# justinkay/coda

Hardware: NVIDIA H100
Metric: acquisition steps/sec (M=256,N=5e5,C=100) (higher is better)
Workload: dtype f32

## Files before the change

coda_b200/_native.py:

```python
from __future__ import annotations

import ctypes as C
import os
import sys

from . import build as _build

_LIB = None

OK = 0
VERSION = 202
MAX_WORLD = 16
REC_WORDS = 8
FLAG_NONFINITE_INPUT = 0x01
FLAG_RANGE_INPUT = 0x02
FLAG_NONFINITE_TABLE = 0x04
FLAG_NONFINITE_PI = 0x08
FLAG_NONFINITE_PBEST = 0x10
FLAG_NONFINITE_EIG = 0x20
FLAG_NO_CANDIDATE = 0x40
FLAG_XCHG_TIMEOUT = 0x80
FLAG_NEGATIVE_PROB = 0x100
FLAG_ROWSUM_WARN = 0x200
FLAG_PIPELINE_TIMEOUT = 0x400
FLAG_NAMES = {
    FLAG_NONFINITE_INPUT: "preds", FLAG_RANGE_INPUT: "preds range", FLAG_NONFINITE_TABLE: "pdf/cdf/integrand",
    FLAG_NONFINITE_PI: "pi_hat_xi", FLAG_NONFINITE_PBEST: "Pbest", FLAG_NONFINITE_EIG: "Pbest(beta) normalized",
}

p, i32, i64, f64, f32, sz = C.c_void_p, C.c_int, C.c_int64, C.c_double, C.c_float, C.c_size_t


class XchgStruct(C.Structure):
    _fields_ = [("world", i32), ("rank", i32), ("box", p * MAX_WORLD), ("epoch", p), ("H", i32), ("C", i32),
                ("rep_words", i32)]


class StepStruct(C.Structure):
    _fields_ = [
        ("H", i32), ("C", i32), ("N", i64), ("n_offset", i64), ("fx_shift", i32), ("lr", f32),
        ("hard", p), ("labeled", p), ("D", p), ("jvec", p), ("sel", p),
        ("terms", p), ("slot_of_model", p), ("shadow_off", i64), ("shadow_col_stride", i64), ("model_stride", i64),
        ("have_ens", i32), ("compact_k", i32),
        ("pisum_fx", p), ("PB", p), ("pi_hat", p), ("m0", p), ("h_before", p), ("best_model", p),
        ("partials", p), ("nblocks", i32), ("eig", p), ("bestrec", p),
        ("labels_global", p), ("hist_idx", p), ("hist_q", p), ("hist_tie", p), ("hist_cap", i64), ("step_ctr", p),
        ("flags", p),
    ]


PX, PS = C.POINTER(XchgStruct), C.POINTER(StepStruct)

SIGNATURES = {
    "coda_b200_last_error": (C.c_char_p, []),
    "coda_b200_version": (i32, []),
    "coda_b200_sm_count": (i32, []),
    "coda_b200_device_check": (i32, []),
    "coda_b200_set_l2_fetch_granularity": (i32, [i32]),
    "coda_b200_xchg_box_bytes": (sz, [i32, i32, i32, i32]),
    "coda_b200_xchg_alloc": (i32, [sz, C.POINTER(p)]),
    "coda_b200_xchg_free": (i32, [p]),
    "coda_b200_ipc_export": (i32, [p, p]),
    "coda_b200_ipc_open": (i32, [p, C.POINTER(p)]),
    "coda_b200_ipc_close": (i32, [p]),
    "coda_b200_peer_enable": (i32, [i32]),
    "coda_b200_scan_slab": (i32, [p, i64, i32, i64, i32, p, p, p, p, p, p]),
    "coda_b200_confusion_accum": (i32, [p, i64, p, i32, i64, i32, i32, p, p]),
    "coda_b200_confusion_sorted": (i32, [p, i64, p, p, i32, i64, i32, i32, p, p]),
    "coda_b200_init_dirichlets": (i32, [p, p, i32, i32, i32, f64, f64, i32, p, p]),
    "coda_b200_scan_compact": (i32, [p, p, i64, i32, i64, i32, i32, p, p, p, p, p, p]),
    "coda_b200_confusion_compact": (i32, [p, p, i64, p, i32, i64, i32, i32, i32, p, p, p]),
    "coda_b200_pi_full_compact": (i32, [p, p, i64, p, i32, i64, i32, i32, p, p, p, p]),
    "coda_b200_pi_rank1_compact": (i32, [p, p, i64, p, i32, i64, i32, i32, p, f64, i32, p, p, p, p, p]),
    "coda_b200_compact_index_count": (i32, [p, i64, i32, i64, i32, i32, p, p]),
    "coda_b200_compact_index_fill": (i32, [p, p, i64, i32, i64, i32, i32, p, p, p, p]),
    "coda_b200_pi_rank1_index": (i32, [p, p, p, p, i32, i64, i32, p, f64, i32, p, p, p, p, p, p]),
# ... 87 lines not shown
```

coda_b200/csrc/slab.cu:

```cuda
#include "common.cuh"
#include "terms.cuh"

#include <stdlib.h>

__global__ void __launch_bounds__(256) k_scan_slab(const float* __restrict__ preds, long long ldh, int H, long long N, int C,
                                                   int TN, uint16_t* __restrict__ hard,
                                                   int32_t* __restrict__ pseudo, uint8_t* __restrict__ disagree,
                                                   float* __restrict__ ens_out, uint32_t* __restrict__ flags) {
  extern __shared__ __align__(16) unsigned char smem_raw[];
  float* ens = reinterpret_cast<float*>(smem_raw);
  uint16_t* hard_t = reinterpret_cast<uint16_t*>(ens + (size_t)TN * C);
  const int warp = threadIdx.x >> 5, lane = threadIdx.x & 31, nwarp = blockDim.x >> 5;
  const long long n0 = (long long)blockIdx.x * TN;
  const int tn = (int)min((long long)TN, N - n0);
  for (int i = threadIdx.x; i < TN * C; i += blockDim.x) ens[i] = 0.f;
  __syncthreads();
  uint32_t bad = 0;
  for (int h = 0; h < H; ++h) {
    const float* base = preds + (size_t)h * ldh + (size_t)n0 * C;
    for (int p = warp; p < tn; p += nwarp) {
      const float* row = base + (size_t)p * C;
      float* erow = ens + (size_t)p * C;
      float bv = -INFINITY;
      int bi = 0x7fffffff;
// ... 542 lines not shown
    for (int k = 0; k < KC; ++k) {
      const int c = lane + 32 * k;
      u[r][k] = (ok && c < C) ? urow[c] : 0.f;
    }
  }
#pragma unroll
  for (int r = 0; r < NR; ++r) {
    if (r * rstride >= nrows) break;
    float* urow = U + (size_t)(row0 + r * rstride) * C;
    float s = 0.f;
#pragma unroll
    for (int k = 0; k < KC; ++k) {
      const int c = lane + 32 * k;
      if (c == t) {
        u[r][k] += dv[r];
        urow[c] = u[r][k];
      }
      s += u[r][k];
    }
    s = warp_sum(s);
    if (!isfinite(s)) bad |= CODA_B200_FLAG_NONFINITE_PI;
    const float den = fmaxf(s, 1e-12f);
    const float rden = 1.0f / den;
#pragma unroll
    for (int k = 0; k < KC; ++k) racc[k] += to_fx(row_quot(u[r][k], den, rden), fxs);
  }
}

#define R1_CONST_TERMS 3584
__constant__ R1Term c_terms_bank[R1_CONST_TERMS];

#define R1_TN 256
template <int KC, int GU = 16, int NR = 4, bool CONST_TERMS = false>
__global__ void __launch_bounds__(256, (GU > 16 ? 3 : 4)) k_pi_rank1(const float* __restrict__ preds, const float* __restrict__ E,
                                                  long long N, int C, const long long* __restrict__ sel,
                                                  const int32_t* __restrict__ hdr, const R1Term* __restrict__ gterms,
                                                  int const_base, float lr, float fxs,
                                                  float* __restrict__ U, unsigned long long* __restrict__ pisum_fx,
                                                  uint32_t* __restrict__ flags) {
  extern __shared__ __align__(16) unsigned char smem_raw[];
  long long* wacc_all = reinterpret_cast<long long*>(smem_raw);
  R1Term* s_terms = reinterpret_cast<R1Term*>(wacc_all + (size_t)8 * C);
  const int warp = threadIdx.x >> 5, lane = threadIdx.x & 31;
  const int t = (int)sel[1];
  const int nt = hdr[0], tp = hdr[1];
  if (!CONST_TERMS)
    for (int k = threadIdx.x; k < nt; k += blockDim.x) s_terms[k] = gterms[k];
  const R1Term* c_terms = CONST_TERMS ? (c_terms_bank + const_base) : s_terms;
  long long* wacc = wacc_all + (size_t)warp * C;
  for (int c = lane; c < C; c += 32) wacc[c] = 0;
  long long racc[KC > 0 ? KC : 1];
#pragma unroll
  for (int k = 0; k < (KC > 0 ? KC : 1); ++k) racc[k] = 0;
  __syncthreads();
  uint32_t bad = 0;
  const long long wstride = (long long)gridDim.x * R1_TN;
  for (long long n0 = (long long)blockIdx.x * R1_TN + warp * 32; n0 < N; n0 += wstride) {
    const long long n = n0 + lane;
    float d = 0.f;
    if (n < N) {
      if (tp >= 0) d = __ldg(E + (size_t)n * C + tp);
      int k = 0;
      for (; k + GU <= nt; k += GU) {
        float v[GU];
#pragma unroll
        for (int q = 0; q < GU; ++q) v[q] = __ldg(preds + c_terms[k + q].off + n * c_terms[k + q].str);
#pragma unroll
        for (int q = 0; q < GU; ++q) d = fmaf(c_terms[k + q].sg, v[q], d);
      }
      for (; k < nt; ++k) d = fmaf(c_terms[k].sg, __ldg(preds + c_terms[k].off + n * c_terms[k].str), d);
    }
    const float dl = lr * d;
    const int rows = (int)min(32LL, N - n0);
    if (KC > 0) {
      for (int r = 0; r < rows; r += NR) {
        float dv[NR];
#pragma unroll
        for (int i = 0; i < NR; ++i) dv[i] = __shfl_sync(CODA_FULL, dl, (r + i) & 31);
        rows_accumulate_reg<(KC > 0 ? KC : 1), NR>(U, n0 + r, rows - r, 1, C, lane, fxs, t, dv, racc, bad);
      }
    } else {
      for (int r = 0; r < rows; ++r) {
        const float dr = __shfl_sync(CODA_FULL, dl, r);
        row_accumulate(U + (size_t)(n0 + r) * C, C, lane, fxs, t, dr, nullptr, wacc, bad);
      }
    }
  }
  if (KC > 0) {
#pragma unroll
    for (int k = 0; k < (KC > 0 ? KC : 1); ++k) {
      const int c = lane + 32 * k;
      if (c < C) wacc[c] = racc[k];
    }
  }
  __syncthreads();
  for (int c = threadIdx.x; c < C; c += blockDim.x) {
    long long s2 = 0;
    for (int w = 0; w < 8; ++w) s2 += wacc_all[(size_t)w * C + c];
    if (s2) atomicAdd(pisum_fx + c, (unsigned long long)s2);
  }
  if (bad) atomicOr(flags, bad);
}

#define R1V_WI 128
template <int KC>
__global__ void __launch_bounds__(256, 3) k_pi_rank1_v4(const float* __restrict__ preds, const float* __restrict__ E,
                                                     long long N, int C, const long long* __restrict__ sel,
                                                     const int32_t* __restrict__ hdr, const R1Term* __restrict__ gterms,
                                                     float lr, float fxs, float* __restrict__ U,
                                                     unsigned long long* __restrict__ pisum_fx,
                                                     uint32_t* __restrict__ flags) {
  extern __shared__ __align__(16) unsigned char smem_raw[];
  long long* wacc_all = reinterpret_cast<long long*>(smem_raw);
  R1Term* c_terms = reinterpret_cast<R1Term*>(wacc_all + (size_t)8 * C);
  const int warp = threadIdx.x >> 5, lane = threadIdx.x & 31;
  const int t = (int)sel[1];
  const int nt = hdr[0], tp = hdr[1];
  for (int k = threadIdx.x; k < nt; k += blockDim.x) c_terms[k] = gterms[k];
  long long racc[KC];
#pragma unroll
  for (int k = 0; k < KC; ++k) racc[k] = 0;
  __syncthreads();
  uint32_t bad = 0;
  const long long cta_items = (long long)8 * R1V_WI;
  for (long long n0 = (long long)blockIdx.x * cta_items + (long long)warp * R1V_WI; n0 < N; n0 += (long long)gridDim.x * cta_items) {
    const long long nl = n0 + 4 * lane;
    const bool full4 = nl + 3 < N;
    float d[4] = {0.f, 0.f, 0.f, 0.f};
    if (tp >= 0) {
#pragma unroll
      for (int i = 0; i < 4; ++i)
        if (nl + i < N) d[i] = __ldg(E + (size_t)(nl + i) * C + tp);
    }
    int k = 0;
    for (; k + 8 <= nt; k += 8) {
      float v[8][4];
#pragma unroll
      for (int q = 0; q < 8; ++q) {
        const R1Term tm = c_terms[k + q];
        if (tm.str == 1 && full4) {
          const float4 x = __ldg(reinterpret_cast<const float4*>(preds + tm.off + nl));
          v[q][0] = x.x; v[q][1] = x.y; v[q][2] = x.z; v[q][3] = x.w;
        } else {
#pragma unroll
          for (int i = 0; i < 4; ++i) v[q][i] = (nl + i < N) ? __ldg(preds + tm.off + (nl + i) * tm.str) : 0.f;
        }
      }
#pragma unroll
      for (int q = 0; q < 8; ++q) {
        const float sg = c_terms[k + q].sg;
#pragma unroll
        for (int i = 0; i < 4; ++i) d[i] = fmaf(sg, v[q][i], d[i]);
      }
    }
    for (; k < nt; ++k) {
      const R1Term tm = c_terms[k];
#pragma unroll
      for (int i = 0; i < 4; ++i) {
        const float x = (nl + i < N) ? __ldg(preds + tm.off + (nl + i) * tm.str) : 0.f;
        d[i] = fmaf(tm.sg, x, d[i]);
      }
    }
    float dl[4];
#pragma unroll
    for (int i = 0; i < 4; ++i) dl[i] = lr * d[i];
    const int rows = (int)min((long long)R1V_WI, N - n0);
    for (int r = 0; r < rows; r += 4) {
      float dv[4];
#pragma unroll
      for (int i = 0; i < 4; ++i) dv[i] = __shfl_sync(CODA_FULL, dl[i], r >> 2);
      rows_accumulate_reg<KC, 4>(U, n0 + r, rows - r, 1, C, lane, fxs, t, dv, racc, bad);
    }
  }
  long long* wacc = wacc_all + (size_t)warp * C;
#pragma unroll
  for (int k = 0; k < KC; ++k) {
    const int c = lane + 32 * k;
    if (c < C) wacc[c] = racc[k];
  }
  __syncthreads();
  for (int c = threadIdx.x; c < C; c += blockDim.x) {
    long long s2 = 0;
    for (int w = 0; w < 8; ++w) s2 += wacc_all[(size_t)w * C + c];
    if (s2) atomicAdd(pisum_fx + c, (unsigned long long)s2);
  }
  if (bad) atomicOr(flags, bad);
}

#define R1X_THREADS 320
#define R1X_ST 4
#define R1X_TB 16

template <int KC>
__global__ void __launch_bounds__(R1X_THREADS, 1) k_pi_rank1_tma(const float* __restrict__ preds,
                                                                 const float* __restrict__ E, long long N, int C, int TR,
                                                                 const long long* __restrict__ sel,
                                                                 const int32_t* __restrict__ hdr,
                                                                 const R1Term* __restrict__ gterms, float lr, float fxs,
                                                                 float* __restrict__ U,
                                                                 unsigned long long* __restrict__ pisum_fx,
                                                                 uint32_t* __restrict__ flags) {
  extern __shared__ __align__(128) unsigned char smem_r1x[];
  unsigned char* smem_raw = smem_r1x;
  const int nt = hdr[0], tp = hdr[1];
  const int t = (int)sel[1];
  const size_t u_bytes = ((size_t)TR * C * 4 + 127) & ~(size_t)127;
  float* Ut = reinterpret_cast<float*>(smem_raw);
  float* ring = reinterpret_cast<float*>(smem_raw + u_bytes);
  R1Term* terms = reinterpret_cast<R1Term*>(ring + (size_t)R1X_ST * R1X_TB * TR);
  long long* wacc_all = reinterpret_cast<long long*>(terms + nt);
  int* shl = reinterpret_cast<int*>(wacc_all + (size_t)8 * C);
  uint64_t* bars = reinterpret_cast<uint64_t*>((reinterpret_cast<uintptr_t>(shl + nt) + 7) & ~(uintptr_t)7);
  uint64_t* fullU = bars, *emptyU = bars + 1, *full = bars + 2, *empty = bars + 2 + R1X_ST;
  __shared__ int s_nsh;
  const int tid = threadIdx.x, warp = tid >> 5, lane = tid & 31;
  const int nwarp_act = TR >> 5;
  for (int k = tid; k < nt; k += R1X_THREADS) terms[k] = gterms[k];
  for (int c = tid; c < 8 * C; c += R1X_THREADS) wacc_all[c] = 0;
  if (tid == 0) {
    mbar_init(fullU, 1);
    mbar_init(emptyU, nwarp_act);
    for (int s = 0; s < R1X_ST; ++s) { mbar_init(&full[s], 1); mbar_init(&empty[s], nwarp_act); }
    mbar_fence_init();
  }
  __syncthreads();
  if (tid == 0) {
    int n = 0;
    for (int k = 0; k < nt; ++k)
      if (terms[k].str == 1) shl[n++] = k;
    s_nsh = n;
  }
  __syncthreads();
  const int nsh = s_nsh;
  const int nch = (nsh + R1X_TB - 1) / R1X_TB;
  const long long ntiles = (N + TR - 1) / TR;

  if (warp == 8) {
// ... 12 lines not shown
            tma_load_1d(ring + ((size_t)s * R1X_TB + j) * TR, preds + terms[shl[c * R1X_TB + j]].off + n0, rb, &full[s]);
        }
      }
    }
    return;
  }
  if (warp == 9) {
    if (lane == 0) {
      long long it = 0;
      for (long long ti = blockIdx.x; ti < ntiles; ti += gridDim.x, ++it) {
        const long long n0 = ti * TR;
        const int rows = (int)min((long long)TR, N - n0);
        const uint32_t ub = ((uint32_t)rows * C * 4u + 15u) & ~15u;
        if (it > 0) mbar_wait(emptyU, (uint32_t)((it - 1) & 1));
        mbar_expect_tx(fullU, ub);
        tma_load_1d(Ut, U + (size_t)n0 * C, ub, fullU);
      }
    }
    return;
  }
  if (warp >= nwarp_act) return;
  long long racc[KC];
#pragma unroll
  for (int k = 0; k < KC; ++k) racc[k] = 0;
  uint32_t bad = 0;
  long long gch = 0, it = 0;
  for (long long ti = blockIdx.x; ti < ntiles; ti += gridDim.x, ++it) {
    const long long n0 = ti * TR;
    const int rows = (int)min((long long)TR, N - n0);
    const int li = warp * 32 + lane;
    const long long n = n0 + li;
    const bool valid = li < rows;
    float d = 0.f;
    if (valid && tp >= 0) d = __ldg(E + (size_t)n * C + tp);
    int shi = 0;
    const float* slot = ring;
    for (int k = 0; k < nt; ++k) {
      const R1Term tm = terms[k];
      float v = 0.f;
      if (tm.str == 1) {
        const int j = shi % R1X_TB;
        if (j == 0) {
          const long long g = gch + shi / R1X_TB;
          const int s = (int)(g % R1X_ST);
          mbar_wait(&full[s], (uint32_t)((g / R1X_ST) & 1));
          slot = ring + (size_t)s * R1X_TB * TR;
        }
        v = slot[(size_t)j * TR + li];
        ++shi;
        if (j == R1X_TB - 1 || shi == nsh) {
          __syncwarp();
          if (lane == 0) mbar_arrive(&empty[(int)((gch + (shi - 1) / R1X_TB) % R1X_ST)]);
        }
      } else if (valid) {
        v = __ldg(preds + tm.off + n * tm.str);
      }
      d = fmaf(tm.sg, v, d);
    }
    gch += nch;
    const float dl = valid ? lr * d : 0.f;
    mbar_wait(fullU, (uint32_t)(it & 1));
    const int wrows = min(32, rows - warp * 32);
    for (int r = 0; r < wrows; r += 4) {
      float u[4][KC], dv[4];
#pragma unroll
      for (int i = 0; i < 4; ++i) {
        dv[i] = __shfl_sync(CODA_FULL, dl, (r + i) & 31);
// ... 47 lines not shown
  int tr = (int)((104 * 1024) / ((size_t)C * 4)) / 32 * 32;
  if (tr > 256) tr = 256;
  return tr;
}

extern "C" int coda_b200_pi_rank1(const float* preds, const float* ens, int H, int64_t N, int C, const int64_t* sel,
                                  double lr, int fx_shift, const int32_t* terms , float* U,
                                  int64_t* pisum_fx, uint32_t* flags, int ctas_per_sm, int const_slot,
                                  coda_stream_t stream) {
  CODA_CHECK_ARG(preds && sel && terms && U && pisum_fx && flags, "pi_rank1: null pointer");
  CODA_CHECK_ARG(2 * H <= R1_MAXT, "pi_rank1: H=%d too large", H);
  CODA_CHECK_ARG((reinterpret_cast<uintptr_t>(terms) & 7) == 0, "pi_rank1: terms must be 8-byte aligned");
  const int32_t* hdr = terms;
  const R1Term* tlist = reinterpret_cast<const R1Term*>(terms + 2);
  cudaStream_t st = as_stream(stream);
  const char* r1env = getenv("CODA_B200_R1");
  const bool want_tma = r1env && r1env[0] == 't';
  const bool want_v1 = !(r1env && r1env[0] == 'v' && r1env[1] == '4');
  const bool want_deep = r1env && r1env[0] == 'v' && r1env[1] == '1' && r1env[2] == 'd';
  const bool no_tma = !want_tma;
  const int TR = C <= 128 ? r1x_tile_rows(C) : 0;
  if (!no_tma && TR >= 32 && (reinterpret_cast<uintptr_t>(U) & 15) == 0) {
    const size_t u_bytes = ((size_t)TR * C * 4 + 127) & ~(size_t)127;
    const size_t smem_x = u_bytes + (size_t)R1X_ST * R1X_TB * TR * 4 + (size_t)2 * H * sizeof(R1Term) + (size_t)8 * C * 8 +
                          (size_t)2 * H * 4 + 8 + (2 + 2 * R1X_ST) * 8;
    if (smem_x <= 220 * 1024) {
      long long tiles = (N + TR - 1) / TR;
      int cap = coda_sm_count();
      if (ctas_per_sm >= 1 && ctas_per_sm < 8) cap = cap - cap / 8;
      int gridx = (int)min(tiles, (long long)cap);
#define LAUNCH_R1X(KC)                                                                                              \
  do {                                                                                                              \
    CODA_CUDA_OK(cudaFuncSetAttribute(k_pi_rank1_tma<KC>, cudaFuncAttributeMaxDynamicSharedMemorySize, (int)smem_x)); \
    k_pi_rank1_tma<KC><<<gridx, R1X_THREADS, smem_x, st>>>(preds, ens, N, C, TR, reinterpret_cast<const long long*>(sel), \
                                                          hdr, tlist, (float)lr, exp2f((float)fx_shift), U,        \
                                                          reinterpret_cast<unsigned long long*>(pisum_fx), flags); \
  } while (0)
      if (C <= 32) LAUNCH_R1X(1);
      else if (C <= 64) LAUNCH_R1X(2);
      else LAUNCH_R1X(4);
#undef LAUNCH_R1X
      CODA_LAUNCH_OK("k_pi_rank1_tma");
      return CODA_B200_OK;
    }
  }
  size_t smem = (size_t)8 * C * 8 + (size_t)2 * H * sizeof(R1Term);
  CODA_CHECK_ARG(smem <= 200 * 1024, "pi_rank1: C=%d too large", C);
  if (!want_v1 && C <= 128) {
    long long want4 = (N + 8 * R1V_WI - 1) / (8 * R1V_WI);
    int cps = (ctas_per_sm < 1 || ctas_per_sm > 8) ? 8 : ctas_per_sm;
    int grid4 = (int)min(want4, (long long)coda_sm_count() * cps);
#define LAUNCH_R1V(KC)                                                                                            \
  do {                                                                                                            \
    CODA_CUDA_OK(cudaFuncSetAttribute(k_pi_rank1_v4<KC>, cudaFuncAttributeMaxDynamicSharedMemorySize, (int)smem)); \
    k_pi_rank1_v4<KC><<<grid4, 256, smem, st>>>(preds, ens, N, C, reinterpret_cast<const long long*>(sel), hdr,   \
                                               tlist, (float)lr, exp2f((float)fx_shift), U,                       \
                                               reinterpret_cast<unsigned long long*>(pisum_fx), flags);           \
  } while (0)
    if (C <= 32) LAUNCH_R1V(1);
    else if (C <= 64) LAUNCH_R1V(2);
    else LAUNCH_R1V(4);
#undef LAUNCH_R1V
    CODA_LAUNCH_OK("k_pi_rank1_v4");
    return CODA_B200_OK;
  }
  long long want = (N + R1_TN - 1) / R1_TN;
  if (ctas_per_sm < 1 || ctas_per_sm > 8) ctas_per_sm = 8;
  int grid = (int)min(want, (long long)coda_sm_count() * ctas_per_sm);
  const int slot_terms = (2 * H + 63) / 64 * 64;
  const bool use_const = const_slot >= 0 && (long long)(const_slot + 1) * slot_terms <= R1_CONST_TERMS && C <= 128;
  const int const_base = use_const ? const_slot * slot_terms : 0;
  if (use_const)
    CODA_CUDA_OK(cudaMemcpyToSymbolAsync(c_terms_bank, tlist, (size_t)2 * H * sizeof(R1Term),
                                         (size_t)const_base * sizeof(R1Term), cudaMemcpyDeviceToDevice, st));
#define LAUNCH_R1(KC)                                                                                          \
  do {                                                                                                         \
    if (use_const) {                                                                                           \
      CODA_CUDA_OK(cudaFuncSetAttribute(k_pi_rank1<KC, 16, 4, true>, cudaFuncAttributeMaxDynamicSharedMemorySize, (int)smem)); \
      k_pi_rank1<KC, 16, 4, true><<<grid, 256, smem, st>>>(preds, ens, N, C, reinterpret_cast<const long long*>(sel), hdr, \
                                            tlist, const_base, (float)lr, exp2f((float)fx_shift), U,           \
                                            reinterpret_cast<unsigned long long*>(pisum_fx), flags);           \
      break;                                                                                                   \
    }                                                                                                          \
    CODA_CUDA_OK(cudaFuncSetAttribute(k_pi_rank1<KC>, cudaFuncAttributeMaxDynamicSharedMemorySize, (int)smem)); \
    k_pi_rank1<KC><<<grid, 256, smem, st>>>(preds, ens, N, C, reinterpret_cast<const long long*>(sel), hdr,    \
                                            tlist, 0, (float)lr, exp2f((float)fx_shift), U,                    \
                                            reinterpret_cast<unsigned long long*>(pisum_fx), flags);           \
  } while (0)
  if (want_deep && C > 64 && C <= 128) {
    CODA_CUDA_OK(cudaFuncSetAttribute(k_pi_rank1<4, 32, 8>, cudaFuncAttributeMaxDynamicSharedMemorySize, (int)smem));
    k_pi_rank1<4, 32, 8><<<grid, 256, smem, st>>>(preds, ens, N, C, reinterpret_cast<const long long*>(sel), hdr, tlist, 0,
                                                  (float)lr, exp2f((float)fx_shift), U,
                                                  reinterpret_cast<unsigned long long*>(pisum_fx), flags);
    CODA_LAUNCH_OK("k_pi_rank1<deep>");
    return CODA_B200_OK;
  }
  if (C <= 32) LAUNCH_R1(1);
  else if (C <= 64) LAUNCH_R1(2);
  else if (C <= 128) LAUNCH_R1(4);
  else LAUNCH_R1(0);
#undef LAUNCH_R1
  CODA_LAUNCH_OK("k_pi_rank1");
  return CODA_B200_OK;
}
```

coda_b200/csrc/step.cu:

```cuda
#include "xchg.cuh"
#include "terms.cuh"

#define ST_THREADS 256

__device__ void apply_label(const coda_step_t& a, int t, const int* jv, int* cnt , bool valid) {
  const int H = a.H, C = a.C, tid = threadIdx.x;
  unsigned long long* pz = reinterpret_cast<unsigned long long*>(a.pisum_fx);
  for (int c = tid; c < C; c += ST_THREADS) pz[c] = 0ull;
  int32_t* hdr = a.terms;
  R1Term* terms = reinterpret_cast<R1Term*>(a.terms + 2);
  if (!valid) {
    if (tid == 0) { hdr[0] = 0; hdr[1] = -1; }
    return;
  }
  for (int h = tid; h < H; h += ST_THREADS) {
    a.jvec[h] = jv[h];
    a.D[((size_t)h * C + t) * C + jv[h]] += a.lr;
  }
  __shared__ int s_tp, s_m, s_total;
  __shared__ int wtot[ST_THREADS / 32];
  for (int c = tid; c < C; c += ST_THREADS) cnt[c] = 0;
  __syncthreads();
  for (int h = tid; h < H; h += ST_THREADS) atomicAdd(&cnt[jv[h]], 1);
  __syncthreads();
  if (tid == 0) {
    int best = -1, bc = 0;
    for (int c = 0; c < C; ++c)
      if (cnt[c] > best) { best = cnt[c]; bc = c; }
    s_tp = bc;
    s_m = H - best;
  }
  __syncthreads();
  const int tp = s_tp, M = s_m;
  const bool ens = a.have_ens && 2 * M < H;
  int carry = 0;
  const int lane = tid & 31, warp = tid >> 5;
  for (int h0 = 0; h0 < H; h0 += ST_THREADS) {
    const int h = h0 + tid;
    const int j = h < H ? jv[h] : 0;
    const int n = h < H ? (ens ? (j != tp ? 2 : 0) : 1) : 0;
    int incl = n;
#pragma unroll
    for (int o = 1; o < 32; o <<= 1) {
      const int v = __shfl_up_sync(CODA_FULL, incl, o);
      if (lane >= o) incl += v;
    }
    if (lane == 31) wtot[warp] = incl;
    __syncthreads();
    int off = carry;
    for (int w = 0; w < warp; ++w) off += wtot[w];
    const int k = off + incl - n;
    if (n && a.compact_k > 0) {
      terms[k] = R1Term{(long long)h, 1.f, j};
      if (n == 2) terms[k + 1] = R1Term{(long long)h, -1.f, tp};
    } else if (n) {
      const int slot = a.slot_of_model ? a.slot_of_model[h] : -1;
      const long long base = slot >= 0 ? a.shadow_off + (long long)slot * C * a.shadow_col_stride : (long long)h * a.model_stride;
      const long long mul = slot >= 0 ? a.shadow_col_stride : 1;
      const int str = slot >= 0 ? 1 : C;
      terms[k] = R1Term{base + (long long)j * mul, 1.f, str};
      if (n == 2) terms[k + 1] = R1Term{base + (long long)tp * mul, -1.f, str};
    }
    if (tid == ST_THREADS - 1) s_total = off + incl;
    __syncthreads();
    carry = s_total;
  }
  if (tid == 0) {
    hdr[0] = carry;
// ... 403 lines not shown
```

coda_b200/engine.py:

```python
from __future__ import annotations

import contextlib
import math
import os

import numpy as np
import torch

from . import _native as nat

_CONST_SLOTS = {}
_CONST_TERMS = 3584


def _acquire_const_slot(dev_index, H):
    per = (2 * H + 63) // 64 * 64
    used = _CONST_SLOTS.setdefault(dev_index, set())
    for s in range(_CONST_TERMS // per):
        if s not in used:
            used.add(s)
            return s
    return -1


def _release_const_slot(dev_index, slot):
    if slot is not None and slot >= 0:
        _CONST_SLOTS.get(dev_index, set()).discard(slot)


TIE_CAP = 256
REP_WORDS = 12 + TIE_CAP + TIE_CAP // 2
MODES = ("incremental", "recompute", "recompute_all")
TABLE_BATCH_BYTES = 512 << 20
HIST_CAP = 1 << 16


def _ptr(t):
    return t.data_ptr() if t is not None else None


class Engine:
    rep_words = REP_WORDS

    def __init__(self, preds: torch.Tensor, *, alpha: float, learning_rate: float, multiplier: float,
                 uniform_prior: bool, hyp_w: float = 1.0, mode: str = "incremental", n_offset: int = 0,
                 n_global: int | None = None, world: int = 1, own_stream: bool = False):
        from .datasets import CompactSlab
        if mode not in MODES:
            raise ValueError(f"mode must be one of {MODES}")
        self.compact = preds if isinstance(preds, CompactSlab) else None
        if not ((isinstance(preds, torch.Tensor) or self.compact is not None) and preds.is_cuda):
            raise RuntimeError("coda_b200: dataset.preds must live on a CUDA (sm_90a) device; "
                               "there is no CPU path in this package")
        H, N, Cc = (int(s) for s in preds.shape)
        if N < 1:
            raise ValueError("coda_b200: empty shard (fewer items than shards?)")
        if self.compact is not None:
            if mode == "recompute_all":
                raise NotImplementedError("coda_b200: mode='recompute_all' is not offered for a compact slab")
            self.K = self.compact.K
        else:
            if preds.dtype != torch.float32 or preds.dim() != 3:
                raise TypeError("coda_b200: preds must be a float32 (H, N, C) tensor (coda/datasets.py:14)")
            if not (preds.stride(2) == 1 and preds.stride(1) == Cc and (H == 1 or preds.stride(0) >= N * Cc)):
                raise ValueError("coda_b200: preds must be (H, N, C) with contiguous items (an N-range view of a "
                                 "contiguous slab is fine)")
        self.lib = nat.load()
        self.preds = preds
        self.dev = preds.device
        with torch.cuda.device(self.dev):
            nat.require_device()
# ... 117 lines not shown
        self.partials = self._z((self.nblocks, nat.REC_WORDS), torch.int64)
        self.rep = self._z((REP_WORDS,), torch.int64)
        self.flags = self.rep[0:1].view(torch.int32)[0:1]
        self.bestrec = self.rep[1:9]
        self.tie_hdr = self.rep[9:11]
        self.tie_idx = self.rep[12:12 + TIE_CAP]
        self.tie_val = self.rep[12 + TIE_CAP:].view(torch.float32)[:TIE_CAP]
        self.rep_all = self._z((self.world, REP_WORDS), torch.int64)
        self.rep_host = torch.zeros((self.world, REP_WORDS), dtype=torch.int64).pin_memory()
        self.sel = self._z((2,), torch.int64)
        self.sel_ring = torch.zeros((8, 2), dtype=torch.int64).pin_memory()
        self.sel_events = [None] * 8
        self.sel_pos = 0
        self.jvec = self._z((H,), torch.int32)
        self.terms = self._z((2 + 8 * H + 2,), torch.int64).view(torch.int32)[: 2 + 8 * H]
        self.step_ctr = self._z((1,), torch.int64)
        self.hist_idx = self._z((HIST_CAP,), torch.int64)
        self.hist_q = self._z((HIST_CAP,), torch.float32)
        self.hist_tie = self._z((HIST_CAP,), torch.int32)
        self.ens = self._e((N, C), torch.float32) if (os.environ.get("CODA_B200_ENS", "1") != "0" or self.compact is not None) else None
        cls_per_batch = max(1, min(C, TABLE_BATCH_BYTES // max(1, self.lib.coda_b200_tables_scratch_bytes(H, 1))))
        self.table_batch = int(cls_per_batch)
        self.scratch = self._e((int(self.lib.coda_b200_tables_scratch_bytes(H, self.table_batch)),), torch.uint8)

    def _make_step_struct(self):
        st = nat.StepStruct()
        st.H, st.C, st.N, st.n_offset, st.fx_shift, st.lr = self.H, self.C, self.N, self.n_offset, self.fx_shift, self.lr
        st.hard, st.labeled, st.D, st.jvec, st.sel = _ptr(self.hard), _ptr(self.labeled), _ptr(self.D), _ptr(self.jvec), _ptr(self.sel)
        st.terms = _ptr(self.terms)
        st.slot_of_model = _ptr(self.slot_of_model)
        st.shadow_off = ((self.shadow.data_ptr() - self._slab_ptr()) // 4) if self.shadow is not None else 0
        st.shadow_col_stride = self.shadow_cs
        st.model_stride = self.model_stride
        st.have_ens = 1 if self.ens is not None else 0
        st.compact_k = self.K if self.compact is not None else 0
        st.pisum_fx, st.PB, st.pi_hat, st.m0 = _ptr(self.pisum), _ptr(self.PB), _ptr(self.pi_hat), _ptr(self.m0)
        st.h_before, st.best_model = _ptr(self.hb), _ptr(self.best_model)
        st.partials, st.nblocks, st.eig, st.bestrec = _ptr(self.partials), self.nblocks, _ptr(self.eig), _ptr(self.bestrec)
        st.labels_global = None
        st.hist_idx, st.hist_q, st.hist_tie, st.hist_cap = _ptr(self.hist_idx), _ptr(self.hist_q), _ptr(self.hist_tie), HIST_CAP
        st.step_ctr = _ptr(self.step_ctr)
        st.flags = _ptr(self.flags)
        self.st = st

    def _slab_ptr(self):
        return self.preds.data_ptr() if self.compact is None else 0

    def _x(self):
        return self.xchg if (self.xchg is not None and self.world > 1) else None

    def construct_scan(self):
        with self._on():
            H, N, C, s = self.H, self.N, self.C, self._s()
            if self.compact is not None:
                cs = self.compact
                self._call("coda_b200_scan_compact", _ptr(cs.ids), _ptr(cs.probs), self.model_stride, H, N, C, self.K,
                           _ptr(self.hard), _ptr(self.pseudo), _ptr(self.disagree), _ptr(self.ens), _ptr(self.flags), s)
                self._call("coda_b200_confusion_compact", _ptr(cs.ids), _ptr(cs.probs), self.model_stride,
                           _ptr(self.pseudo), H, N, C, self.K, self.fx_shift, _ptr(self.conf_fx), _ptr(self.conf_rest), s)
                self._build_compact_index()
                return
            self._call("coda_b200_scan_slab", _ptr(self.preds), self.model_stride, H, N, C, _ptr(self.hard),
                       _ptr(self.pseudo), _ptr(self.disagree), _ptr(self.ens), _ptr(self.flags), s)
            if C <= 128:
                order = torch.argsort(self.pseudo).to(torch.int32)
                self._call("coda_b200_confusion_sorted", _ptr(self.preds), self.model_stride, _ptr(self.pseudo),
                           _ptr(order), H, N, C, self.fx_shift, _ptr(self.conf_fx), s)
                del order
            else:
                self._call("coda_b200_confusion_accum", _ptr(self.preds), self.model_stride, _ptr(self.pseudo), H, N, C,
                           self.fx_shift, _ptr(self.conf_fx), s)

    def construct_posterior(self):
        with self._on():
            H, C, s = self.H, self.C, self._s()
            self._call("coda_b200_init_dirichlets", _ptr(self.conf_fx), _ptr(self.conf_rest), H, C, self.fx_shift,
                       self.prior_strength, self.multiplier, int(self.uniform_prior), _ptr(self.D), s)
            self.conf_fx = self.conf_rest = self.conf_buf = None
            self._marginals_full()
            self._build_rows()
            self._build_shadow()
            self._make_step_struct()
            self._tables(0, C)
            self.cache_valid = False
            self.pending = False
            self.scored = False
            self.reported = False

    def construct_mixture(self):
        with self._on():
            self._mixture()

    def construct_finish(self):
        with self._on():
            self.check_flags(sync=True)

    def _build_compact_index(self):
        self.cidx = None
        if os.environ.get("CODA_B200_COMPACT_INDEX", "1") == "0":
            return
        H, N, C, K, s = self.H, self.N, self.C, self.K, self._s()
        need = 8 * H * N * K + 16 * (H * C + 1) + 12 * N
        free, _total = torch.cuda.mem_get_info(self.dev)
        if need > 0.5 * free:
            return
        cs = self.compact
        counts = self._z((H * C,), torch.int64)
        self._call("coda_b200_compact_index_count", _ptr(cs.ids), self.model_stride, H, N, C, K, _ptr(counts), s)
        off = self._z((H * C + 1,), torch.int64)
        torch.cumsum(counts, 0, out=off[1:])
        cursor = off[:-1].clone()
        ent = self._e((H * N * K,), torch.int64)
        rest = self._e((N,), torch.float32)
        self._call("coda_b200_compact_index_fill", _ptr(cs.ids), _ptr(cs.probs), self.model_stride, H, N, C, K,
                   _ptr(cursor), _ptr(ent), _ptr(rest), s, n=2)
        del counts, cursor
# ... 66 lines not shown
        self.tile_off_host = tile_off
        self.tile_off = torch.from_numpy(tile_off).to(self.dev)
        self.ntiles = int(tile_off[-1])
        self.ent_row = self._e((max(1, n_ent),), torch.int32)
        self.ent_cls = self._e((max(1, n_ent),), torch.int16)
        self.zmask = self._e((self.npairs, W), torch.int32)
        self.row_of = self._e((self.npairs,), torch.int32)
        self.row_cls = self._e((max(1, self.n_heavy),), torch.int16)
        cursor = self._z((C,), torch.int32)
        self._call("coda_b200_pair_fill", _ptr(self.hard), H, N, C, _ptr(self.ent_off), _ptr(self.heavy_off),
                   _ptr(self.cls_base), _ptr(cursor), _ptr(self.ent_row), _ptr(self.ent_cls), _ptr(self.zmask),
                   _ptr(self.row_of), _ptr(self.row_cls), s, n=2)
        self.ell_row, self.ell_cls, self.ell_k = None, None, 0
        if 0 < self.max_entries <= 32 and C <= 128:
            self.ell_k = (self.max_entries + 3) // 4 * 4
            self.ell_row = self._e((N, self.ell_k), torch.int32)
            self.ell_cls = self._e((N, self.ell_k), torch.int16)
            self._call("coda_b200_ell_build", _ptr(self.ent_off), _ptr(self.ent_row), _ptr(self.ent_cls), N, self.ell_k,
                       _ptr(self.ell_row), _ptr(self.ell_cls), s)
        self.gain = self._z((self.npairs,), torch.float32)
        self.fused_score = os.environ.get("CODA_B200_FUSED_SCORE", "0") == "1"
        self.ph_cache = None
        if self.mode == "incremental":
            need = self.npairs * self.Hp * 4
            free, _total = torch.cuda.mem_get_info(self.dev)
            if need + (2 << 30) > free + torch.cuda.memory_reserved(self.dev) - torch.cuda.memory_allocated(self.dev):
                import warnings
                warnings.warn(f"coda_b200: row cache of {need / 2 ** 30:.1f} GiB does not fit "
                              f"({free / 2 ** 30:.1f} GiB free); falling back to mode='recompute'")
                self.mode = "recompute"
            else:
                self.ph_cache = self._e((self.npairs, self.Hp), torch.float32)

    def _build_shadow(self):
        self.shadow, self.slot_of_model, self.n_shadow, self.shadow_cs = None, None, 0, 0
        if self.mode == "recompute_all" or os.environ.get("CODA_B200_SHADOW", "1") == "0" or self.compact is not None:
            return
        H, N, C = self.H, self.N, self.C
        cs = (N + 3) // 4 * 4
        torch.cuda.synchronize(self.dev)
        torch.cuda.empty_cache()
        free, _total = torch.cuda.mem_get_info(self.dev)
        reserve = int(float(os.environ.get("CODA_B200_SHADOW_RESERVE_GB", "8")) * 2 ** 30)
        per_model = cs * C * 4
        S = int(min(H, max(0, (free - reserve) // per_model)))
        cap = os.environ.get("CODA_B200_SHADOW_MODELS")
        if cap is not None:
            S = min(S, int(cap))
        if S <= 0:
            return
        dis = torch.zeros(H, dtype=torch.int64, device=self.dev)
        step = max(1, (64 << 20) // max(1, H))
        for n0 in range(0, N, step):
            blk = self.hard[n0:n0 + step].to(torch.int32) & 0xFFFF
            dis += (blk != self.pseudo[n0:n0 + step, None]).sum(0)
        order = torch.argsort(dis, descending=True, stable=True)[:S].to(torch.int32)
        slot = torch.full((H,), -1, dtype=torch.int32, device=self.dev)
        slot[order.long()] = torch.arange(S, dtype=torch.int32, device=self.dev)
        self.shadow = self._e((S, C, cs), torch.float32)
        self._call("coda_b200_shadow_build", _ptr(self.preds), self.model_stride, H, N, C, _ptr(order), S, cs,
                   _ptr(self.shadow), self._s())
        self.slot_of_model, self.n_shadow, self.shadow_cs = slot, S, cs

    def _tables(self, lo, hi, sel=False):
        H, C, s = self.H, self.C, self._s()
        if sel:
            self._call("coda_b200_beta_tables", _ptr(self.D), _ptr(self.grid), H, C, self.P, self.hyp_w, 0, 1,
                       _ptr(self.sel), _ptr(self.scratch), _ptr(self.dL), _ptr(self.G0T), _ptr(self.G1T),
                       _ptr(self.PB), _ptr(self.dLb), _ptr(self.Gb), _ptr(self.flags), s, n=3)
            return
        for b0 in range(lo, hi, self.table_batch):
            b1 = min(hi, b0 + self.table_batch)
            self._call("coda_b200_beta_tables", _ptr(self.D), _ptr(self.grid), H, C, self.P, self.hyp_w, b0, b1, None,
                       _ptr(self.scratch), _ptr(self.dL), _ptr(self.G0T), _ptr(self.G1T), _ptr(self.PB),
                       _ptr(self.dLb), _ptr(self.Gb), _ptr(self.flags), s, n=3)

    def _mixture(self):
        self._call("coda_b200_step_mixture", self.st, self._x(), self._s())

    def _pair_rows(self, tile_lo, tile_hi, gains=True, sel=False):
        tail = (_ptr(self.PB), _ptr(self.m0) if gains else None, _ptr(self.pi_hat) if gains else None, self.H,
                _ptr(self.ph_cache), _ptr(self.gain) if gains else None, _ptr(self.sel) if sel else None,
                _ptr(self.tile_off) if sel else None, _ptr(self.flags), self._s())
        if self.use_tc:
            self._call("coda_b200_pair_rows_tc", _ptr(self.tiles), int(tile_lo), int(tile_hi), _ptr(self.zmask),
                       _ptr(self.row_of), _ptr(self.dLb), _ptr(self.Gb), *tail)
        else:
            self._call("coda_b200_pair_rows", _ptr(self.tiles), int(tile_lo), int(tile_hi), _ptr(self.zmask),
                       _ptr(self.row_of), _ptr(self.dL), _ptr(self.G0T), _ptr(self.G1T), *tail)

    def _score(self):
        if self.scored:
            return
        if self.mode == "incremental":
# ... 297 lines not shown
            return xi

    def state_tensors(self):
        return {"D": self.D, "U": self.U, "labeled": self.labeled, "pisum": self.pisum, "step_ctr": self.step_ctr}

    def __del__(self):
        try:
            _release_const_slot(self.dev.index, getattr(self, "const_slot", -1))
        except Exception:
            pass

    def close(self):
        self.graphs.clear()
        _release_const_slot(self.dev.index, self.const_slot)
        self.const_slot = -1
        if self._mailbox is not None:
            self._mailbox.close()
            self._mailbox = None
        for k, v in list(self.__dict__.items()):
            if isinstance(v, torch.Tensor) or k in ("preds", "compact", "st", "xchg", "_labels_keep", "cidx"):
                setattr(self, k, None)


def build_engines(shards, group, **kw):
    n_global = kw.pop("n_global")
    own = len(shards) > 1
    engines = [Engine(p, n_offset=off, n_global=n_global, world=group.world, own_stream=own, **kw) for p, off in shards]
    for e in engines:
        e.construct_scan()
    group.attach(engines)
    group.allreduce_sum_([e.conf_buf for e in engines])
    for e in engines:
        e.construct_posterior()
    for e in engines:
        e.construct_mixture()
    for e in engines:
        e.construct_finish()
    return engines
```

include/coda_b200.h:

```cpp
#ifndef CODA_B200_H
#define CODA_B200_H

#include <stddef.h>
#include <stdint.h>

#ifdef __cplusplus
extern "C" {
#endif

#define CODA_B200_VERSION 202
#define CODA_B200_NODES 256
#define CODA_B200_MAX_WORLD 16
#define CODA_B200_REC_WORDS 8

#define CODA_B200_OK 0
#define CODA_B200_EINVAL (-1)
#define CODA_B200_ECUDA (-2)

#define CODA_B200_FLAG_NONFINITE_INPUT 0x01u
#define CODA_B200_FLAG_RANGE_INPUT 0x02u
#define CODA_B200_FLAG_NONFINITE_TABLE 0x04u
#define CODA_B200_FLAG_NONFINITE_PI 0x08u
#define CODA_B200_FLAG_NONFINITE_PBEST 0x10u
#define CODA_B200_FLAG_NONFINITE_EIG 0x20u
// ... 100 lines not shown
                        const int64_t* tile_off , uint32_t* flags, coda_stream_t stream);
int coda_b200_pair_rows_tc(const int32_t* tiles128, int tile_lo, int tile_hi, const uint32_t* zmask,
                           const int32_t* row_of, const void* dLb, const void* Gb, const float* PB, const float* m0,
                           const float* pi_hat, int H, float* ph_cache, float* gain, const int64_t* sel,
                           const int64_t* tile_off, uint32_t* flags, coda_stream_t stream);
int coda_b200_template_gains(const float* ph_cache, int H, int C, const float* PB, const float* m0,
                             const float* pi_hat, float* gain , coda_stream_t stream);

int coda_b200_eig_blocks(int64_t N, int H, int C);
int coda_b200_gain_eig(const float* U, int64_t N, int C, int H, const int32_t* ent_off, const int32_t* heavy_off,
                       const int32_t* ent_row, const uint16_t* ent_cls, const float* ph_cache, const float* gain,
                       const float* PB, const float* m0, const float* pi_hat, const uint8_t* labeled,
                       const uint8_t* disagree, int64_t n_offset, int max_entries, const int32_t* ell_row,
                       const uint16_t* ell_cls, int ell_k, float* eig, int64_t* partials, uint32_t* flags,
                       coda_stream_t stream);
int coda_b200_ell_build(const int32_t* ent_off, const int32_t* ent_row, const uint16_t* ent_cls, int64_t N, int K,
                        int32_t* ell_row , uint16_t* ell_cls , coda_stream_t stream);
int coda_b200_row_gains(const float* ph_cache, const uint16_t* row_cls, int64_t n_heavy, int H, int C,
                        const float* PB, const float* m0, const float* pi_hat, float* gain, coda_stream_t stream);

typedef struct coda_step {
  int H, C;
  int64_t N, n_offset;
  int fx_shift;
  float lr;
  const uint16_t* hard;
  uint8_t* labeled;
  float* D;
  int32_t* jvec;
  int64_t* sel;
  int32_t* terms;
  const int32_t* slot_of_model;
  int64_t shadow_off, shadow_col_stride, model_stride;
  int have_ens;
  int compact_k;
  int64_t* pisum_fx;
  const float* PB;
  float* pi_hat;
  float* m0;
  float* h_before;
  int64_t* best_model;
  const int64_t* partials;
  int nblocks;
  const float* eig;
  int64_t* bestrec;
  const int64_t* labels_global;
  int64_t* hist_idx;
  float* hist_q;
  int32_t* hist_tie;
  int64_t hist_cap;
  int64_t* step_ctr;
  uint32_t* flags;
} coda_step_t;

int coda_b200_step_select(const coda_step_t* st, const coda_xchg_t* x, coda_stream_t stream);
int coda_b200_step_merge(const coda_step_t* st, const coda_xchg_t* x, coda_stream_t stream);
int coda_b200_step_label(const coda_step_t* st, const coda_xchg_t* x, coda_stream_t stream);
int coda_b200_step_mixture(const coda_step_t* st, const coda_xchg_t* x, coda_stream_t stream);

int coda_b200_ties(const float* eig, int64_t N, const uint8_t* labeled, const uint8_t* disagree, int64_t n_offset,
                   const int64_t* best , int cap, int64_t* tie_hdr , int64_t* tie_idx,
                   float* tie_val, coda_stream_t stream);
int coda_b200_report_gather(const int64_t* rep, int rep_words, int64_t* rep_all, const coda_xchg_t* x,
                            uint32_t* flags, coda_stream_t stream);


// ... 20 lines not shown
```

Baseline: 560.2.

## Fold ensemble column into rank-1 term list via column-major shadow slot

```diff
diff --git a/coda_b200/_native.py b/coda_b200/_native.py
--- a/coda_b200/_native.py
+++ b/coda_b200/_native.py
@@ -41,7 +41,7 @@
         ("H", i32), ("C", i32), ("N", i64), ("n_offset", i64), ("fx_shift", i32), ("lr", f32),
         ("hard", p), ("labeled", p), ("D", p), ("jvec", p), ("sel", p),
         ("terms", p), ("slot_of_model", p), ("shadow_off", i64), ("shadow_col_stride", i64), ("model_stride", i64),
-        ("have_ens", i32), ("compact_k", i32),
+        ("ens_off", i64), ("ens_col_stride", i64), ("have_ens", i32), ("compact_k", i32),
         ("pisum_fx", p), ("PB", p), ("pi_hat", p), ("m0", p), ("h_before", p), ("best_model", p),
         ("partials", p), ("nblocks", i32), ("eig", p), ("bestrec", p),
         ("labels_global", p), ("hist_idx", p), ("hist_q", p), ("hist_tie", p), ("hist_cap", i64), ("step_ctr", p),
diff --git a/coda_b200/csrc/slab.cu b/coda_b200/csrc/slab.cu
--- a/coda_b200/csrc/slab.cu
+++ b/coda_b200/csrc/slab.cu
@@ -598,8 +598,7 @@
 
 #define R1_TN 256
 template <int KC, int GU = 16, int NR = 4, bool CONST_TERMS = false>
-__global__ void __launch_bounds__(256, (GU > 16 ? 3 : 4)) k_pi_rank1(const float* __restrict__ preds, const float* __restrict__ E,
-                                                  long long N, int C, const long long* __restrict__ sel,
+__global__ void __launch_bounds__(256, (GU > 16 ? 3 : 4)) k_pi_rank1(const float* __restrict__ preds, long long N, int C, const long long* __restrict__ sel,
                                                   const int32_t* __restrict__ hdr, const R1Term* __restrict__ gterms,
                                                   int const_base, float lr, float fxs,
                                                   float* __restrict__ U, unsigned long long* __restrict__ pisum_fx,
@@ -609,7 +608,7 @@
   R1Term* s_terms = reinterpret_cast<R1Term*>(wacc_all + (size_t)8 * C);
   const int warp = threadIdx.x >> 5, lane = threadIdx.x & 31;
   const int t = (int)sel[1];
-  const int nt = hdr[0], tp = hdr[1];
+  const int nt = hdr[0];
   if (!CONST_TERMS)
     for (int k = threadIdx.x; k < nt; k += blockDim.x) s_terms[k] = gterms[k];
   const R1Term* c_terms = CONST_TERMS ? (c_terms_bank + const_base) : s_terms;
@@ -625,7 +624,6 @@
     const long long n = n0 + lane;
     float d = 0.f;
     if (n < N) {
-      if (tp >= 0) d = __ldg(E + (size_t)n * C + tp);
       int k = 0;
       for (; k + GU <= nt; k += GU) {
         float v[GU];
@@ -670,8 +668,7 @@
 
 #define R1V_WI 128
 template <int KC>
-__global__ void __launch_bounds__(256, 3) k_pi_rank1_v4(const float* __restrict__ preds, const float* __restrict__ E,
-                                                     long long N, int C, const long long* __restrict__ sel,
+__global__ void __launch_bounds__(256, 3) k_pi_rank1_v4(const float* __restrict__ preds, long long N, int C, const long long* __restrict__ sel,
                                                      const int32_t* __restrict__ hdr, const R1Term* __restrict__ gterms,
                                                      float lr, float fxs, float* __restrict__ U,
                                                      unsigned long long* __restrict__ pisum_fx,
@@ -681,7 +678,7 @@
   R1Term* c_terms = reinterpret_cast<R1Term*>(wacc_all + (size_t)8 * C);
   const int warp = threadIdx.x >> 5, lane = threadIdx.x & 31;
   const int t = (int)sel[1];
-  const int nt = hdr[0], tp = hdr[1];
+  const int nt = hdr[0];
   for (int k = threadIdx.x; k < nt; k += blockDim.x) c_terms[k] = gterms[k];
   long long racc[KC];
 #pragma unroll
@@ -693,11 +690,6 @@
     const long long nl = n0 + 4 * lane;
     const bool full4 = nl + 3 < N;
     float d[4] = {0.f, 0.f, 0.f, 0.f};
-    if (tp >= 0) {
-#pragma unroll
-      for (int i = 0; i < 4; ++i)
-        if (nl + i < N) d[i] = __ldg(E + (size_t)(nl + i) * C + tp);
-    }
     int k = 0;
     for (; k + 8 <= nt; k += 8) {
       float v[8][4];
@@ -759,7 +751,7 @@
 
 template <int KC>
 __global__ void __launch_bounds__(R1X_THREADS, 1) k_pi_rank1_tma(const float* __restrict__ preds,
-                                                                 const float* __restrict__ E, long long N, int C, int TR,
+                                                                 long long N, int C, int TR,
                                                                  const long long* __restrict__ sel,
                                                                  const int32_t* __restrict__ hdr,
                                                                  const R1Term* __restrict__ gterms, float lr, float fxs,
@@ -768,7 +760,7 @@
                                                                  uint32_t* __restrict__ flags) {
   extern __shared__ __align__(128) unsigned char smem_r1x[];
   unsigned char* smem_raw = smem_r1x;
-  const int nt = hdr[0], tp = hdr[1];
+  const int nt = hdr[0];
   const int t = (int)sel[1];
   const size_t u_bytes = ((size_t)TR * C * 4 + 127) & ~(size_t)127;
   float* Ut = reinterpret_cast<float*>(smem_raw);
@@ -847,7 +839,6 @@
     const long long n = n0 + li;
     const bool valid = li < rows;
     float d = 0.f;
-    if (valid && tp >= 0) d = __ldg(E + (size_t)n * C + tp);
     int shi = 0;
     const float* slot = ring;
     for (int k = 0; k < nt; ++k) {
@@ -961,7 +952,7 @@
 #define LAUNCH_R1X(KC)                                                                                              \
   do {                                                                                                              \
     CODA_CUDA_OK(cudaFuncSetAttribute(k_pi_rank1_tma<KC>, cudaFuncAttributeMaxDynamicSharedMemorySize, (int)smem_x)); \
-    k_pi_rank1_tma<KC><<<gridx, R1X_THREADS, smem_x, st>>>(preds, ens, N, C, TR, reinterpret_cast<const long long*>(sel), \
+    k_pi_rank1_tma<KC><<<gridx, R1X_THREADS, smem_x, st>>>(preds, N, C, TR, reinterpret_cast<const long long*>(sel), \
                                                           hdr, tlist, (float)lr, exp2f((float)fx_shift), U,        \
                                                           reinterpret_cast<unsigned long long*>(pisum_fx), flags); \
   } while (0)
@@ -982,7 +973,7 @@
 #define LAUNCH_R1V(KC)                                                                                            \
   do {                                                                                                            \
     CODA_CUDA_OK(cudaFuncSetAttribute(k_pi_rank1_v4<KC>, cudaFuncAttributeMaxDynamicSharedMemorySize, (int)smem)); \
-    k_pi_rank1_v4<KC><<<grid4, 256, smem, st>>>(preds, ens, N, C, reinterpret_cast<const long long*>(sel), hdr,   \
+    k_pi_rank1_v4<KC><<<grid4, 256, smem, st>>>(preds, N, C, reinterpret_cast<const long long*>(sel), hdr,   \
                                                tlist, (float)lr, exp2f((float)fx_shift), U,                       \
                                                reinterpret_cast<unsigned long long*>(pisum_fx), flags);           \
   } while (0)
@@ -1006,19 +997,19 @@
   do {                                                                                                         \
     if (use_const) {                                                                                           \
       CODA_CUDA_OK(cudaFuncSetAttribute(k_pi_rank1<KC, 16, 4, true>, cudaFuncAttributeMaxDynamicSharedMemorySize, (int)smem)); \
-      k_pi_rank1<KC, 16, 4, true><<<grid, 256, smem, st>>>(preds, ens, N, C, reinterpret_cast<const long long*>(sel), hdr, \
+      k_pi_rank1<KC, 16, 4, true><<<grid, 256, smem, st>>>(preds, N, C, reinterpret_cast<const long long*>(sel), hdr, \
                                             tlist, const_base, (float)lr, exp2f((float)fx_shift), U,           \
                                             reinterpret_cast<unsigned long long*>(pisum_fx), flags);           \
       break;                                                                                                   \
     }                                                                                                          \
     CODA_CUDA_OK(cudaFuncSetAttribute(k_pi_rank1<KC>, cudaFuncAttributeMaxDynamicSharedMemorySize, (int)smem)); \
-    k_pi_rank1<KC><<<grid, 256, smem, st>>>(preds, ens, N, C, reinterpret_cast<const long long*>(sel), hdr,    \
+    k_pi_rank1<KC><<<grid, 256, smem, st>>>(preds, N, C, reinterpret_cast<const long long*>(sel), hdr,    \
                                             tlist, 0, (float)lr, exp2f((float)fx_shift), U,                    \
                                             reinterpret_cast<unsigned long long*>(pisum_fx), flags);           \
   } while (0)
   if (want_deep && C > 64 && C <= 128) {
     CODA_CUDA_OK(cudaFuncSetAttribute(k_pi_rank1<4, 32, 8>, cudaFuncAttributeMaxDynamicSharedMemorySize, (int)smem));
-    k_pi_rank1<4, 32, 8><<<grid, 256, smem, st>>>(preds, ens, N, C, reinterpret_cast<const long long*>(sel), hdr, tlist, 0,
+    k_pi_rank1<4, 32, 8><<<grid, 256, smem, st>>>(preds, N, C, reinterpret_cast<const long long*>(sel), hdr, tlist, 0,
                                                   (float)lr, exp2f((float)fx_shift), U,
                                                   reinterpret_cast<unsigned long long*>(pisum_fx), flags);
     CODA_LAUNCH_OK("k_pi_rank1<deep>");
diff --git a/coda_b200/csrc/step.cu b/coda_b200/csrc/step.cu
--- a/coda_b200/csrc/step.cu
+++ b/coda_b200/csrc/step.cu
@@ -33,7 +33,12 @@
   __syncthreads();
   const int tp = s_tp, M = s_m;
   const bool ens = a.have_ens && 2 * M < H;
-  int carry = 0;
+  const bool ens_term = ens && a.compact_k == 0;
+  if (ens_term && tid == 0) {
+    const bool cm = a.ens_col_stride > 0;
+    terms[0] = R1Term{a.ens_off + (long long)tp * (cm ? a.ens_col_stride : 1), 1.f, cm ? 1 : C};
+  }
+  int carry = ens_term ? 1 : 0;
   const int lane = tid & 31, warp = tid >> 5;
   for (int h0 = 0; h0 < H; h0 += ST_THREADS) {
     const int h = h0 + tid;
diff --git a/coda_b200/engine.py b/coda_b200/engine.py
--- a/coda_b200/engine.py
+++ b/coda_b200/engine.py
@@ -37,6 +37,12 @@
 
 def _ptr(t):
     return t.data_ptr() if t is not None else None
+
+
+def shadow_slots(free: int, reserve: int, slot_bytes: int, want: int, ens: bool, left: int = 1, total: int = 1):
+    n = max(0, (free - total * reserve) // max(1, left) // slot_bytes)
+    ne = 1 if ens and n >= 1 else 0
+    return int(max(0, min(want, n - ne))), ne
 
 
 class Engine:
@@ -220,6 +226,12 @@
         st.shadow_off = ((self.shadow.data_ptr() - self._slab_ptr()) // 4) if self.shadow is not None else 0
         st.shadow_col_stride = self.shadow_cs
         st.model_stride = self.model_stride
+        if self.shadow is not None and self.shadow.shape[0] > self.n_shadow:
+            st.ens_off = (self.shadow[self.n_shadow].data_ptr() - self._slab_ptr()) // 4
+            st.ens_col_stride = self.shadow_cs
+        else:
+            st.ens_off = ((self.ens.data_ptr() - self._slab_ptr()) // 4) if self.ens is not None else 0
+            st.ens_col_stride = 0
         st.have_ens = 1 if self.ens is not None else 0
         st.compact_k = self.K if self.compact is not None else 0
         st.pisum_fx, st.PB, st.pi_hat, st.m0 = _ptr(self.pisum), _ptr(self.PB), _ptr(self.pi_hat), _ptr(self.m0)
@@ -267,9 +279,12 @@
             self.conf_fx = self.conf_rest = self.conf_buf = None
             self._marginals_full()
             self._build_rows()
-            self._build_shadow()
+
+    def construct_tables(self, left: int = 1, total: int = 1):
+        with self._on():
+            self._build_shadow(left, total)
             self._make_step_struct()
-            self._tables(0, C)
+            self._tables(0, self.C)
             self.cache_valid = False
             self.pending = False
             self.scored = False
@@ -402,34 +417,46 @@
             else:
                 self.ph_cache = self._e((self.npairs, self.Hp), torch.float32)
 
-    def _build_shadow(self):
+    def shadow_reserve(self) -> int:
+        env = os.environ.get("CODA_B200_SHADOW_RESERVE_GB")
+        if env is not None:
+            return int(float(env) * 2 ** 30)
+        return 4 * self.N * self.C + (1 << 30)
+
+    def _build_shadow(self, left: int = 1, total: int = 1):
         self.shadow, self.slot_of_model, self.n_shadow, self.shadow_cs = None, None, 0, 0
         if self.mode == "recompute_all" or os.environ.get("CODA_B200_SHADOW", "1") == "0" or self.compact is not None:
             return
         H, N, C = self.H, self.N, self.C
         cs = (N + 3) // 4 * 4
+        cap = os.environ.get("CODA_B200_SHADOW_MODELS")
+        want = H if cap is None else max(0, min(H, int(cap)))
+        order = None
+        if want > 0:
+            dis = torch.zeros(H, dtype=torch.int64, device=self.dev)
+            step = max(1, (64 << 20) // max(1, H))
+            for n0 in range(0, N, step):
+                blk = self.hard[n0:n0 + step].to(torch.int32) & 0xFFFF
+                dis += (blk != self.pseudo[n0:n0 + step, None]).sum(0)
+            order = torch.argsort(dis, descending=True, stable=True).to(torch.int32)
+            del dis, blk
         torch.cuda.synchronize(self.dev)
         torch.cuda.empty_cache()
         free, _total = torch.cuda.mem_get_info(self.dev)
-        reserve = int(float(os.environ.get("CODA_B200_SHADOW_RESERVE_GB", "8")) * 2 ** 30)
-        per_model = cs * C * 4
-        S = int(min(H, max(0, (free - reserve) // per_model)))
-        cap = os.environ.get("CODA_B200_SHADOW_MODELS")
-        if cap is not None:
-            S = min(S, int(cap))
-        if S <= 0:
+        S, ne = shadow_slots(free, self.shadow_reserve(), cs * C * 4, want, self.ens is not None, left, total)
+        if S + ne == 0:
             return
-        dis = torch.zeros(H, dtype=torch.int64, device=self.dev)
-        step = max(1, (64 << 20) // max(1, H))
-        for n0 in range(0, N, step):
-            blk = self.hard[n0:n0 + step].to(torch.int32) & 0xFFFF
-            dis += (blk != self.pseudo[n0:n0 + step, None]).sum(0)
-        order = torch.argsort(dis, descending=True, stable=True)[:S].to(torch.int32)
         slot = torch.full((H,), -1, dtype=torch.int32, device=self.dev)
-        slot[order.long()] = torch.arange(S, dtype=torch.int32, device=self.dev)
-        self.shadow = self._e((S, C, cs), torch.float32)
-        self._call("coda_b200_shadow_build", _ptr(self.preds), self.model_stride, H, N, C, _ptr(order), S, cs,
-                   _ptr(self.shadow), self._s())
+        self.shadow = self._e((S + ne, C, cs), torch.float32)
+        if S > 0:
+            order = order[:S].contiguous()
+            slot[order.long()] = torch.arange(S, dtype=torch.int32, device=self.dev)
+            self._call("coda_b200_shadow_build", _ptr(self.preds), self.model_stride, H, N, C, _ptr(order), S, cs,
+                       _ptr(self.shadow), self._s())
+        if ne:
+            first = torch.zeros(1, dtype=torch.int32, device=self.dev)
+            self._call("coda_b200_shadow_build", _ptr(self.ens), N * C, 1, N, C, _ptr(first), 1, cs,
+                       _ptr(self.shadow[S]), self._s())
         self.slot_of_model, self.n_shadow, self.shadow_cs = slot, S, cs
 
     def _tables(self, lo, hi, sel=False):
@@ -793,6 +820,13 @@
     group.allreduce_sum_([e.conf_buf for e in engines])
     for e in engines:
         e.construct_posterior()
+    total = {}
+    for e in engines:
+        total[e.dev] = total.get(e.dev, 0) + 1
+    left = dict(total)
+    for e in engines:
+        e.construct_tables(left[e.dev], total[e.dev])
+        left[e.dev] -= 1
     for e in engines:
         e.construct_mixture()
     for e in engines:
diff --git a/include/coda_b200.h b/include/coda_b200.h
--- a/include/coda_b200.h
+++ b/include/coda_b200.h
@@ -156,6 +156,7 @@
   int32_t* terms;
   const int32_t* slot_of_model;
   int64_t shadow_off, shadow_col_stride, model_stride;
+  int64_t ens_off, ens_col_stride;
   int have_ens;
   int compact_k;
   int64_t* pisum_fx;
```

Result: faster. 640.9, median of 6 (+14.4%).
